# adr-arroyo/PointCloudComparator

Measured on NVIDIA B200. Metric: knn_queries_per_s_k16_10M, higher is better.
Workload: dtype f32

## Files before the change

### pointcloudcomparator_b200/csrc/pcc_knn.cu

```cuda
#include <algorithm>
#include <cmath>
#include <cstring>

#include <cub/device/device_select.cuh>
#include <cub/iterator/counting_input_iterator.cuh>

#include "pcc_internal.h"
#include "pcc_fastknn.cuh"

namespace pcc {

__device__ __forceinline__ bool load_query(const Grid &g, const QueryView &v, int64_t t, float &x, float &y, float &z, int64_t &row, bool &write_empty) {
    write_empty = false;
    if (t >= v.nq) return false;
    if (v.self) { row = rows_query(g, v, t, x, y, z); return true; }
    row = rows_query(g, v, t, x, y, z);
#ifdef PCC_EXP_SEQROWS
    row = t;
#endif
#ifdef PCC_EXP_SEQQ
    { float4 p = __ldg(v.q + t); x = p.x; y = p.y; z = p.z; }
#endif
    if (!finite3(x, y, z) || g.n == 0) { write_empty = true; return false; }
    return true;
}

template <class List>
__device__ __forceinline__ void knn_search(const Grid &g, float x, float y, float z, int k, List &list) {
    const QueryCell c = locate(g, x, y, z);
    int Rin = -1, R = 1;
    for (;;) {
        scan_progressive(g, c, Rin, R, [&]() { return to_cell_units(g, key_d2(list.at(k - 1))); },
                         [&](uint32_t, float4 p) { list.offer(make_key(dist2(x, y, z, p.x, p.y, p.z), __float_as_uint(p.w))); });
        const float cov = covered_d2(g, c, R);
        if (cov == CUDART_INF_F) break;
        const nkey_t kth = list.at(k - 1);
        if (kth != PCC_EMPTY_KEY && key_d2(kth) < cov) break;
        Rin = R; R = next_ring(g, R, key_d2(kth));
    }
}

template <int K>
__device__ __forceinline__ void write_row(const nkey_t (&key)[K], int k, int32_t *__restrict__ oi, float *__restrict__ od, int vec4) {
    if (vec4 && K >= 4 && k == K) {
#pragma unroll
        for (int j = 0; j + 3 < K; j += 4) {
            reinterpret_cast<int4 *>(oi)[j >> 2] = make_int4(key_idx(key[j]), key_idx(key[j + 1]), key_idx(key[j + 2]), key_idx(key[j + 3]));
            reinterpret_cast<float4 *>(od)[j >> 2] = make_float4(key_d2(key[j]), key_d2(key[j + 1]), key_d2(key[j + 2]), key_d2(key[j + 3]));
        }
    } else {
#pragma unroll
        for (int j = 0; j < K; ++j) if (j < k) { oi[j] = key_idx(key[j]); od[j] = key_d2(key[j]); }
    }
}
template <int K>
__device__ __forceinline__ void knn_reg_body(const Grid &g, const QueryView &v, int64_t t, int k, int32_t *__restrict__ out_idx, float *__restrict__ out_d2, int vec4) {
    float x, y, z; int64_t row; bool empty;
    RegList<K> list; list.init();
    const bool live = load_query(g, v, t, x, y, z, row, empty);
    if (!live && !empty) return;
    if (live) knn_search(g, x, y, z, k, list);
    write_row<K>(list.key, k, out_idx + row * k, out_d2 + row * k, vec4);
}
template <int K>
__global__ void __launch_bounds__(128) knn_reg_kernel(Grid g, QueryView v, int k, int32_t *__restrict__ out_idx, float *__restrict__ out_d2, int vec4) {
    knn_reg_body<K>(g, v, (int64_t)blockIdx.x * blockDim.x + threadIdx.x, k, out_idx, out_d2, vec4);
}
constexpr unsigned kTiedToWide = 4096;
struct FixList { uint32_t *list; unsigned *count; unsigned long long *stats; uint32_t *ring_list; unsigned *ring_count; uint8_t *ring_flag; uint32_t *wide_list; unsigned *wide_count; uint32_t *late_list; unsigned *late_count; uint32_t *retry_list; unsigned *retry_count; };
__device__ __forceinline__ void push_list(uint32_t *list, unsigned *count, uint32_t value) {
    const unsigned mask = __activemask();
    const int leader = __ffs(mask) - 1, lane = threadIdx.x & 31;
    unsigned base = 0;
    if (lane == leader) base = atomicAdd(count, (unsigned)__popc(mask));
    base = __shfl_sync(mask, base, leader);
    list[base + __popc(mask & ((1u << lane) - 1))] = value;
}
template <int K>
__global__ void __launch_bounds__(128) knn_fixup_kernel(Grid g, QueryView v, int k, int32_t *__restrict__ out_idx, float *__restrict__ out_d2, int vec4, FixList fix) {
    const unsigned n = *fix.count;
    if (fix.wide_list && n <= kTiedToWide) return;
    for (unsigned i = blockIdx.x * blockDim.x + threadIdx.x; i < n; i += gridDim.x * blockDim.x) knn_reg_body<K>(g, v, (int64_t)fix.list[i], k, out_idx, out_d2, vec4);
}

#ifndef PCC_LOG16
#define PCC_LOG16 48
#endif
#ifndef PCC_MB16
#define PCC_MB16 9
#endif
#ifndef PCC_LOG32
#define PCC_LOG32 80
#endif
#ifndef PCC_MB32
#define PCC_MB32 5
#endif
constexpr int64_t kSmallBatch = 1024, kSmallBatchBigK = 64;
constexpr int kRingMaxR = 3;
template <int K> struct FastCfg { static constexpr int threads = 128, log_slots = K <= 16 ? PCC_LOG16 : PCC_LOG32, min_blocks = K <= 16 ? PCC_MB16 : PCC_MB32; };
}
#include "pcc_knn_thr.cuh"
namespace pcc {
template <int K>
__device__ __forceinline__ float kth_distance(const Grid &g, const QueryCell &c, float x, float y, float z, int k, RegDist<K> &list, bool &proved,
                                              uint32_t *__restrict__ slog, int &nlog, const int R0) {
    scan_progressive(g, c, -1, R0, [&]() { return to_cell_units(g, (k == K) ? list.d[K - 1] : list.at(k - 1)); }, [&](uint32_t pos, float4 p) {
        const float d2 = dist2(x, y, z, p.x, p.y, p.z);
        if (d2 <= list.d[K - 1]) {
            if (nlog < FastCfg<K>::log_slots) slog[nlog * FastCfg<K>::threads] = pos;
            ++nlog;
            list.insert(d2);
        }
    });
    const float kth = (k == K) ? list.d[K - 1] : list.at(k - 1);
    const float cov = covered_d2(g, c, R0);
    proved = cov == CUDART_INF_F || kth < cov;
    return kth;
}
template <int K>
__device__ __forceinline__ void knn_fast_body(const Grid &g, const QueryView &v, const int64_t t, int k, int32_t *__restrict__ out_idx, float *__restrict__ out_d2, int vec4,
                                              const FixList &fix, uint32_t *__restrict__ slog, const int R0) {
    constexpr int kFastThreads = FastCfg<K>::threads, kLogSlots = FastCfg<K>::log_slots;
    float x, y, z; int64_t row; bool empty;
    const bool live = load_query(g, v, t, x, y, z, row, empty);
    if (!live) {
        if (R0 == 1 && t < v.nq) fix.ring_flag[t] = 0;
        if (empty) { nkey_t e[K];
#pragma unroll
            for (int j = 0; j < K; ++j) e[j] = PCC_EMPTY_KEY;
            write_row<K>(e, k, out_idx + row * k, out_d2 + row * k, vec4); }
        return;
    }
    const QueryCell c = locate(g, x, y, z);
    RegDist<K> list; list.init();
    int nlog = 0; bool proved;
    const float tau = kth_distance<K>(g, c, x, y, z, k, list, proved, slog, nlog, R0);
    int m = 0;
    if (nlog <= kLogSlots) {
        for (int i = 0; i < nlog; ++i) {
            const uint32_t pos = slog[i * kFastThreads];
            const float4 p = __ldg(g.pts + pos);
            if (dist2(x, y, z, p.x, p.y, p.z) <= tau) { slog[m * kFastThreads] = pos; ++m; }
        }
    } else {
        scan_clipped(g, c, -1, R0, to_cell_units(g, tau), [&](uint32_t pos, float4 p) {
            if (dist2(x, y, z, p.x, p.y, p.z) <= tau) { if (m < kLogSlots) slog[m * kFastThreads] = pos; ++m; }
        });
    }
    if (fix.stats && R0 == 1) { atomicAdd(fix.stats + 0, 1ull); atomicAdd(fix.stats + 1, (unsigned long long)nlog); atomicAdd(fix.stats + 4, proved ? 0ull : 1ull); atomicAdd(fix.stats + 5, m > K ? 1ull : 0ull); atomicAdd(fix.stats + 6, (unsigned long long)m); atomicAdd(fix.stats + 3, nlog > kLogSlots ? 1ull : 0ull); }
    const bool tied = m > K;
    const bool wide = !tied && !proved && (tau == CUDART_INF_F || next_ring(g, 1, tau) > kRingMaxR);
    if (R0 == 1) fix.ring_flag[t] = (!tied && !proved && !wide) ? 1 : 0;
    if (tied) { push_list(fix.list, fix.count, (uint32_t)t); return; }
    if (wide) { push_list(fix.wide_list, fix.wide_count, (uint32_t)t); return; }
    nkey_t e[K];
#pragma unroll
    for (int j = 0; j < K; ++j) {
        e[j] = PCC_EMPTY_KEY;
        if (j < m) { const float4 p = __ldg(g.pts + slog[j * kFastThreads]); e[j] = make_key(dist2(x, y, z, p.x, p.y, p.z), __float_as_uint(p.w)); }
    }
    bitonic_sort_key<K>(e);
    write_row<K>(e, k, out_idx + row * k, out_d2 + row * k, vec4);
}
template <int K>
__global__ void __launch_bounds__(FastCfg<K>::threads, FastCfg<K>::min_blocks) knn_fast_kernel(Grid g, QueryView v, int k, int32_t *__restrict__ out_idx, float *__restrict__ out_d2, int vec4, FixList fix) {
    __shared__ uint32_t slog_all[FastCfg<K>::log_slots * FastCfg<K>::threads];
    knn_fast_body<K>(g, v, (int64_t)blockIdx.x * blockDim.x + threadIdx.x, k, out_idx, out_d2, vec4, fix, slog_all + threadIdx.x, 1);
}
__device__ __forceinline__ nkey_t warp_sort_keys(nkey_t v, int lane) {
#pragma unroll
    for (int size = 2; size <= 32; size <<= 1) {
#pragma unroll
        for (int j = size >> 1; j > 0; j >>= 1) {
            const nkey_t o = __shfl_xor_sync(0xffffffffu, v, j);
            const bool keep_min = ((lane & j) == 0) == ((lane & size) == 0);
            v = (keep_min == (o < v)) ? o : v;
        }
    }
    return v;
}
__device__ __forceinline__ nkey_t warp_merge_keys(nkey_t best, nkey_t batch, int lane) {
    batch = warp_sort_keys(batch, lane);
    const nkey_t r = __shfl_sync(0xffffffffu, batch, 31 - lane);
    nkey_t v = r < best ? r : best;
#pragma unroll
    for (int j = 16; j > 0; j >>= 1) {
        const nkey_t o = __shfl_xor_sync(0xffffffffu, v, j);
        v = (((lane & j) == 0) == (o < v)) ? o : v;
    }
    return v;
}
constexpr int kWideRuns = 64;
__device__ __forceinline__ uint32_t warp_inclusive_scan(uint32_t v, int lane) {
#pragma unroll
    for (int o = 1; o < 32; o <<= 1) { const uint32_t w = __shfl_up_sync(0xffffffffu, v, o); if (lane >= o) v += w; }
    return v;
}
__global__ void __launch_bounds__(128, 5) knn_wide_kernel(Grid g, QueryView v, int k, int32_t *__restrict__ out_idx, float *__restrict__ out_d2, FixList fix,
                                                         const uint32_t *__restrict__ wlist, const unsigned *__restrict__ wcount, int take_tied) {
    __shared__ uint32_t srun_j[4 * kWideRuns], srun_len[4 * kWideRuns], srun_off[4 * (kWideRuns + 1)];
    const int lane = threadIdx.x & 31, wib = threadIdx.x >> 5;
    uint32_t *run_j = srun_j + wib * kWideRuns, *run_len = srun_len + wib * kWideRuns, *run_off = srun_off + wib * (kWideRuns + 1);
    const unsigned n_wide = *wcount, n_tied = (take_tied && *fix.count <= kTiedToWide) ? *fix.count : 0u, n = n_wide + n_tied;
    const unsigned full = 0xffffffffu, lt = (1u << lane) - 1u;
    for (unsigned i = blockIdx.x * 4 + wib; i < n; i += gridDim.x * 4) {
        float x, y, z; int64_t row; bool empty;
        if (!load_query(g, v, (int64_t)(i < n_wide ? wlist[i] : fix.list[i - n_wide]), x, y, z, row, empty)) continue;
        const QueryCell c = locate(g, x, y, z);
        int Rin = -1, R = 3;
        nkey_t best = PCC_EMPTY_KEY;
        float tau = CUDART_INF_F;
        unsigned long long steps = 0;
        for (;;) {
            const int n1 = 2 * R + 1, nrows = n1 * n1;
            const float tau_u = to_cell_units(g, tau);
            const int per = Rin < 0 ? 2 : 1;
            for (int row0 = 0; row0 < nrows; row0 += 32 * per) {
                RowRuns r; r.j1 = r.e1 = r.j2 = r.e2 = 0;
                if (row0 + lane < nrows) r = row_runs(g, c, Rin, R, tau_u, (row0 + lane) / n1, (row0 + lane) % n1);
                if (per == 2 && row0 + 32 + lane < nrows) {
                    const RowRuns r2 = row_runs(g, c, Rin, R, tau_u, (row0 + 32 + lane) / n1, (row0 + 32 + lane) % n1);
                    r.j2 = r2.j1; r.e2 = r2.e1;
                }
                const unsigned m1 = __ballot_sync(full, r.j1 < r.e1), m2 = __ballot_sync(full, r.j2 < r.e2);
                const int nrun = __popc(m1) + __popc(m2);
                if (nrun == 0) continue;
                if (r.j1 < r.e1) { const int q = __popc(m1 & lt); run_j[q] = r.j1; run_len[q] = r.e1 - r.j1; }
                if (r.j2 < r.e2) { const int q = __popc(m1) + __popc(m2 & lt); run_j[q] = r.j2; run_len[q] = r.e2 - r.j2; }
                __syncwarp();
                const uint32_t la = lane < nrun ? run_len[lane] : 0u, lb = lane + 32 < nrun ? run_len[lane + 32] : 0u;
                const uint32_t ia = warp_inclusive_scan(la, lane), ib = warp_inclusive_scan(lb, lane);
                const uint32_t ta = __shfl_sync(full, ia, 31), P = ta + __shfl_sync(full, ib, 31);
                run_off[lane] = ia - la; run_off[lane + 32] = ta + ib - lb;
                if (lane == 0) run_off[kWideRuns] = P;
                __syncwarp();
                int rc = 0;
                for (uint32_t q0 = 0; q0 < P; q0 += 64) {
                    bool has[2] = {false, false}; nkey_t key[2] = {PCC_EMPTY_KEY, PCC_EMPTY_KEY}; float4 p[2];
#pragma unroll
                    for (int u = 0; u < 2; ++u) {
                        const uint32_t q = q0 + 32 * u + lane;
                        has[u] = q < P;
                        if (has[u]) { while (q >= run_off[rc + 1]) ++rc; p[u] = __ldg(g.pts + run_j[rc] + (q - run_off[rc])); }
                    }
#pragma unroll
                    for (int u = 0; u < 2; ++u) {
                        if (has[u]) { const float d2 = dist2(x, y, z, p[u].x, p[u].y, p[u].z); has[u] = d2 <= tau; key[u] = has[u] ? make_key(d2, __float_as_uint(p[u].w)) : PCC_EMPTY_KEY; }
                        if (__ballot_sync(full, has[u])) {
                            best = warp_merge_keys(best, key[u], lane);
                            tau = key_d2(__shfl_sync(full, best, k - 1));
                        }
                    }
                    ++steps;
                }
                __syncwarp();
            }
            const float cov = covered_d2(g, c, R);
            if (cov == CUDART_INF_F || tau < cov) break;
            Rin = R; R = next_ring(g, R, tau);
        }
        if (fix.stats && lane == 0) { atomicAdd(fix.stats + 2, 1ull); atomicAdd(fix.stats + 7, steps); atomicAdd(fix.stats + 8 + (R <= 1 ? 0 : R == 2 ? 1 : R == 3 ? 2 : R < 8 ? 3 : R < 16 ? 4 : 5), 1ull); }
        if (lane < k) { out_idx[row * k + lane] = key_idx(best); out_d2[row * k + lane] = key_d2(best); }
        __syncwarp();
    }
}
constexpr int kRingLog = 24, kRingRuns = 12;
#ifndef PCC_RINGS_MB
#define PCC_RINGS_MB 6
#endif
template <int K>
__global__ void __launch_bounds__(128, K <= 16 ? PCC_RINGS_MB : 4) knn_rings_kernel(Grid g, QueryView v, int k, int32_t *__restrict__ out_idx, float *__restrict__ out_d2, int vec4, FixList fix) {
    __shared__ uint32_t slog_all[kRingLog * 128];
    __shared__ uint2 srun_all[kRingRuns * 128];
    uint32_t *slog = slog_all + threadIdx.x;
    uint2 *srun = srun_all + threadIdx.x;
    const unsigned n = *fix.ring_count;
    for (unsigned i = blockIdx.x * blockDim.x + threadIdx.x; i < n; i += gridDim.x * blockDim.x) {
        const uint32_t t = fix.ring_list[i];
        float x, y, z; int64_t row; bool empty;
        if (!load_query(g, v, (int64_t)t, x, y, z, row, empty)) continue;
        int32_t *oi = out_idx + row * k; float *od = out_d2 + row * k;
        float kth = od[k - 1];
        const QueryCell c = locate(g, x, y, z);
        const int R = kth == CUDART_INF_F ? kRingMaxR + 1 : next_ring(g, 1, kth);
        bool defer = R > kRingMaxR;
        int ncand = 0, nrun = 0, nlog = 0;
        if (!defer) {
            const float tau_u = to_cell_units(g, kth), rad = sqrtf(tau_u) + 2e-3f;
            const int z0 = max(max(c.cz - R, 0), (int)floorf(c.uz - rad)), z1 = min(min(c.cz + R, g.nz - 1), (int)floorf(c.uz + rad));
            const int y0 = max(max(c.cy - R, 0), (int)floorf(c.uy - rad)), y1 = min(min(c.cy + R, g.ny - 1), (int)floorf(c.uy + rad));
            for (int zz = z0; zz <= z1; ++zz) {
                const float gz = fmaxf(fmaxf((float)zz - c.uz, c.uz - (float)(zz + 1)) - 2e-3f, 0.f);
                for (int yy = y0; yy <= y1; ++yy) {
                    const float gy = fmaxf(fmaxf((float)yy - c.uy, c.uy - (float)(yy + 1)) - 2e-3f, 0.f);
                    const float D = gy * gy + gz * gz;
                    if (D > tau_u) continue;
                    const float w = sqrtf(tau_u - D) + 2e-3f;
                    const int xlo = max(max(c.cx - R, 0), (int)floorf(c.ux - w)), xhi = min(min(c.cx + R, g.nx - 1), (int)floorf(c.ux + w));
                    const uint32_t base = (uint32_t)(((size_t)zz * g.ny + yy) * g.nx);
                    const bool shell = max(abs(zz - c.cz), abs(yy - c.cy)) > 1;
                    const int xa1 = xlo, xb1 = shell ? xhi : min(xhi, c.cx - 2);
                    const int xa2 = max(xlo, c.cx + 2), xb2 = shell ? -1 : xhi;
                    if (xa1 <= xb1) { if (ncand < kRingLog) slog[ncand * 128] = (base + (uint32_t)xa1) | ((uint32_t)(xb1 - xa1) << 28); ++ncand; }
                    if (xa2 <= xb2) { if (ncand < kRingLog) slog[ncand * 128] = (base + (uint32_t)xa2) | ((uint32_t)(xb2 - xa2) << 28); ++ncand; }
                }
            }
            defer = ncand > kRingLog;
        }
        if (!defer) {
            for (int r0 = 0; r0 < ncand; r0 += 4) {
                uint32_t cw[4], w0[4], w1[4];
#pragma unroll
                for (int u = 0; u < 4; ++u) {
                    cw[u] = slog[min(r0 + u, ncand - 1) * 128];
                    const uint32_t b = cw[u] & 0x0fffffffu;
                    w0[u] = __ldg(g.occ + (b >> 5)); w1[u] = __ldg(g.occ + (b >> 5) + 1);
                }
#pragma unroll
                for (int u = 0; u < 4; ++u) {
                    const uint32_t b = cw[u] & 0x0fffffffu, len = (cw[u] >> 28) + 1u;
                    const uint32_t bits = __funnelshift_r(w0[u], w1[u], b & 31u) & ((1u << len) - 1u);
                    if (r0 + u < ncand && bits != 0u) { if (nrun < kRingRuns) srun[nrun * 128] = make_uint2(b, b + len); ++nrun; }
                }
            }
            defer = nrun > kRingRuns;
        }
        if (!defer && nrun > 0) {
            for (int r0 = 0; r0 < nrun; r0 += 4) {
                uint2 pr[4];
#pragma unroll
                for (int u = 0; u < 4; ++u) { const uint2 cr = srun[min(r0 + u, nrun - 1) * 128]; pr[u] = make_uint2(__ldg(g.cell_start + cr.x), __ldg(g.cell_start + cr.y)); }
#pragma unroll
                for (int u = 0; u < 4; ++u) if (r0 + u < nrun) srun[(r0 + u) * 128] = pr[u];
            }
            int r = 0;
// ... 397 lines not shown
    p[0] = v.x; p[1] = v.y; p[2] = v.z;
}

__global__ void fill_f32_kernel(float *p, int64_t n, float v) { int64_t i = (int64_t)blockIdx.x * blockDim.x + threadIdx.x; if (i < n) p[i] = v; }

template <int K>
static void launch_knn_reg(const Grid &g, const QueryView &v, int k, int32_t *oi, float *od, int vec4, cudaStream_t s) {
    knn_reg_kernel<K><<<nblocks(v.nq, 128), 128, 0, s>>>(g, v, k, oi, od, vec4);
    PCC_LAUNCHED();
}
template <int K>
static void launch_knn_cell(const Grid &g, const QueryView &v, int k, int32_t *oi, float *od, int vec4, FixList fix, cudaStream_t s) {
    fix.wide_list = nullptr;
    cudaMemsetAsync(fix.count, 0, sizeof(unsigned), s);
    knn_cell_kernel<K><<<nblocks(v.nq, kCellWarps * 32), kCellWarps * 32, 0, s>>>(g, v, k, oi, od, vec4, fix);
    PCC_LAUNCHED();
    knn_fixup_kernel<K><<<148 * 4, 128, 0, s>>>(g, v, k, oi, od, vec4, fix);
    PCC_LAUNCHED();
}
constexpr int64_t kCalibSample = 1 << 15;
constexpr float kCalibQuantile = 0.99f;
template <int K>
static int calibrate_thr(pcc_index *idx, const Grid &g, const QueryView &v, int k, cudaStream_t s) {
    PCC_TRY(idx->calib.reserve((size_t)kCalibBuckets * kCalibBins * 4 + kCalibBuckets * 4));
    unsigned *hist = idx->calib.as<unsigned>();
    float *ratio = (float *)(hist + kCalibBuckets * kCalibBins);
    PCC_CUDA(cudaMemsetAsync(hist, 0, (size_t)kCalibBuckets * kCalibBins * 4, s));
    const int64_t stride = std::max<int64_t>(1, v.nq / kCalibSample), ns = (v.nq + stride - 1) / stride;
    knn_calib_kernel<K><<<nblocks(ns, 128), 128, 0, s>>>(g, v, k, stride, hist);
    PCC_LAUNCHED();
    static const float quantile = getenv("PCC_THR_QUANTILE") ? (float)atof(getenv("PCC_THR_QUANTILE")) : kCalibQuantile;
    knn_calib_finish_kernel<<<1, kCalibBuckets, 0, s>>>(hist, ratio, quantile);
    PCC_LAUNCHED();
    return PCC_OK;
}
template <int K>
static int launch_knn_fast(pcc_index *idx, const Grid &g, const QueryView &v, int k, int32_t *oi, float *od, int vec4, FixList fix, cudaStream_t s) {
    size_t tmp = idx->sel_tmp_bytes;
    if (idx->sel_tmp_nq != v.nq) {
        cub::DeviceSelect::Flagged(nullptr, tmp, cub::CountingInputIterator<uint32_t>(0), fix.ring_flag, fix.ring_list, fix.ring_count, (int)v.nq, s);
        idx->sel_tmp_nq = v.nq; idx->sel_tmp_bytes = tmp;
    }
    PCC_TRY(idx->cub_tmp.reserve(tmp));
    if (!idx->aux_stream) {
        PCC_CUDA(cudaStreamCreateWithFlags(&idx->aux_stream, cudaStreamNonBlocking));
        PCC_CUDA(cudaEventCreateWithFlags(&idx->ev_fork, cudaEventDisableTiming));
        PCC_CUDA(cudaEventCreateWithFlags(&idx->ev_join, cudaEventDisableTiming));
    }
    if (fix.stats) { cudaMemsetAsync(fix.count, 0, sizeof(unsigned), s); cudaMemsetAsync(fix.wide_count, 0, 3 * sizeof(unsigned), s); }
    else cudaMemsetAsync(fix.count, 0, 33 * sizeof(unsigned), s);
    static const bool old_fast_env = getenv("PCC_OLD_FAST") != nullptr;
    static const bool thr_all = getenv("PCC_THR_ALL") != nullptr;
    const bool old_fast = old_fast_env || (K != 16 && !thr_all) || v.nq >= (1ll << 31);
    if (old_fast) {
        knn_fast_kernel<K><<<nblocks(v.nq, FastCfg<K>::threads), FastCfg<K>::threads, 0, s>>>(g, v, k, oi, od, vec4, fix);
        PCC_LAUNCHED();
    } else {
        const pcc_index *owner = idx->grid_owner ? idx->grid_owner : idx;
        unsigned *h_fb = (unsigned *)((char *)idx->h_pinned + 2048);
        if (idx->calib_k == k && idx->calib_gen == owner->grid_gen && idx->calib_nq > 0 && (double)h_fb[0] > 0.04 * (double)idx->calib_nq) idx->calib_k = -1;
        if (idx->calib_k != k || idx->calib_gen != owner->grid_gen) {
            PCC_TRY(calibrate_thr<K>(idx, g, v, k, s));
            idx->calib_k = k; idx->calib_gen = owner->grid_gen;
        }
        const float *ratio = (const float *)(idx->calib.as<unsigned>() + kCalibBuckets * kCalibBins);
        static std::atomic<unsigned long long> attr_done{0};
        if (!((attr_done.load() >> (idx->device & 63)) & 1ull)) {
            PCC_CUDA(cudaFuncSetAttribute(knn_thr_kernel<K, true>, cudaFuncAttributeMaxDynamicSharedMemorySize, (int)ThrCfg<K>::smem));
            PCC_CUDA(cudaFuncSetAttribute(knn_thr_kernel<K, false>, cudaFuncAttributeMaxDynamicSharedMemorySize, (int)ThrCfg<K>::smem));
            PCC_CUDA(cudaFuncSetAttribute(knn_thr_retry_kernel<K, true>, cudaFuncAttributeMaxDynamicSharedMemorySize, (int)ThrCfg<K>::smem));
            PCC_CUDA(cudaFuncSetAttribute(knn_thr_retry_kernel<K, false>, cudaFuncAttributeMaxDynamicSharedMemorySize, (int)ThrCfg<K>::smem));
            attr_done.fetch_or(1ull << (idx->device & 63));
        }
        const char *staged_env = getenv("PCC_THR_STAGED");
        const bool staged = staged_env && atoi(staged_env) != 0;
        if (staged && k == K) {
            static std::atomic<unsigned long long> sattr_done{0};
            if (!((sattr_done.load() >> (idx->device & 63)) & 1ull)) {
                PCC_CUDA(cudaFuncSetAttribute(knn_thr_staged_kernel<K, true>, cudaFuncAttributeMaxDynamicSharedMemorySize, (int)ThrStagedCfg<K>::smem));
                sattr_done.fetch_or(1ull << (idx->device & 63));
            }
            knn_thr_staged_kernel<K, true><<<nblocks(v.nq, ThrCfg<K>::threads), ThrCfg<K>::threads, ThrStagedCfg<K>::smem, s>>>(g, v, k, oi, od, vec4, fix, ratio);
            PCC_LAUNCHED();
            knn_thr_retry_kernel<K, true><<<148 * 4, ThrCfg<K>::threads, ThrCfg<K>::smem, s>>>(g, v, k, oi, od, vec4, fix, ratio);
            PCC_LAUNCHED();
        } else if (k == K) {
            knn_thr_kernel<K, true><<<nblocks(v.nq, ThrCfg<K>::threads), ThrCfg<K>::threads, ThrCfg<K>::smem, s>>>(g, v, k, oi, od, vec4, fix, ratio);
            PCC_LAUNCHED();
            knn_thr_retry_kernel<K, true><<<148 * 4, ThrCfg<K>::threads, ThrCfg<K>::smem, s>>>(g, v, k, oi, od, vec4, fix, ratio);
            PCC_LAUNCHED();
        } else {
            knn_thr_kernel<K, false><<<nblocks(v.nq, ThrCfg<K>::threads), ThrCfg<K>::threads, ThrCfg<K>::smem, s>>>(g, v, k, oi, od, vec4, fix, ratio);
            PCC_LAUNCHED();
            knn_thr_retry_kernel<K, false><<<148 * 4, ThrCfg<K>::threads, ThrCfg<K>::smem, s>>>(g, v, k, oi, od, vec4, fix, ratio);
            PCC_LAUNCHED();
        }
        h_fb[0] = 0; idx->calib_nq = v.nq;
        PCC_CUDA(cudaMemcpyAsync(h_fb, fix.retry_count, sizeof(unsigned), cudaMemcpyDeviceToHost, s));
    }
    PCC_CUDA(cudaEventRecord(idx->ev_fork, s));
    PCC_CUDA(cudaStreamWaitEvent(idx->aux_stream, idx->ev_fork, 0));
    knn_wide_kernel<<<148 * 6, 128, 0, idx->aux_stream>>>(g, v, k, oi, od, fix, fix.wide_list, fix.wide_count, old_fast ? 1 : 0);
    PCC_LAUNCHED();
    PCC_CUDA(cudaEventRecord(idx->ev_join, idx->aux_stream));
    PCC_CUDA(cub::DeviceSelect::Flagged(idx->cub_tmp.p, tmp, cub::CountingInputIterator<uint32_t>(0), fix.ring_flag, fix.ring_list, fix.ring_count, (int)v.nq, s));
    PCC_LAUNCHED();
    knn_rings_kernel<K><<<148 * 16, 128, 0, s>>>(g, v, k, oi, od, vec4, fix);
    PCC_LAUNCHED();
    PCC_CUDA(cudaStreamWaitEvent(s, idx->ev_join, 0));
    knn_wide_kernel<<<148 * 2, 128, 0, s>>>(g, v, k, oi, od, fix, fix.late_list, fix.late_count, 0);
    PCC_LAUNCHED();
    if (old_fast) {
        knn_fixup_kernel<K><<<148 * 4, 128, 0, s>>>(g, v, k, oi, od, vec4, fix);
        PCC_LAUNCHED();
    }
    return PCC_OK;
}

}

using namespace pcc;

static int knn_impl(pcc_index *idx, const void *q, int64_t nq, int stride_bytes, int k, int32_t *out_idx, float *out_d2, int *k_eff, int mem, cudaStream_t s, bool sync) {
    Queries qs;
    PCC_TRY(prepare_queries(idx, q, nq, stride_bytes, mem, s, &qs));
    if (k_eff) *k_eff = (int)std::min<int64_t>(k, idx->n_indexed);
    if (qs.rows == 0) return PCC_OK;
    if (!out_idx || !out_d2) return fail(PCC_ERR_INVALID, "output pointers are NULL");
    int32_t *oi = out_idx; float *od = out_d2;
    const size_t cells = (size_t)qs.rows * k;
    if (mem == PCC_HOST) {
        PCC_TRY(idx->out_i.reserve(cells * 4)); PCC_TRY(idx->out_f.reserve(cells * 4));
        oi = idx->out_i.as<int32_t>(); od = idx->out_f.as<float>();
    }
    if (qs.self && !idx->all_rows_indexed) {
        PCC_CUDA(cudaMemsetAsync(oi, 0xFF, cells * 4, s));
        fill_f32_kernel<<<nblocks((int64_t)cells, 256), 256, 0, s>>>(od, (int64_t)cells, INFINITY);
        PCC_LAUNCHED();
    }
    const Grid g = idx->grid();
    const QueryView v = view_of(qs);
    const int vec4 = ((((uintptr_t)oi) | ((uintptr_t)od)) & 15) == 0 && (k % 4 == 0);
    KernelTimer timer(idx, s);
    if (qs.nq > 0) {
        static const bool exact_env = getenv("PCC_EXACT_ONLY") != nullptr;
        const bool exact_only = exact_env || v.nq < (k <= 32 ? kSmallBatch : kSmallBatchBigK);
        static const bool want_stats = getenv("PCC_STATS") != nullptr;
        const char *cell_env = getenv("PCC_CELL_KERNEL");
        const bool use_cell = cell_env && atoi(cell_env) != 0;
        FixList fix{nullptr, nullptr, nullptr, nullptr, nullptr, nullptr, nullptr, nullptr, nullptr, nullptr, nullptr, nullptr};
        if (k > 1 && k <= 32 && !exact_only) {
            PCC_TRY(idx->misc.reserve((size_t)v.nq * 21 + 512));
            fix.count = idx->misc.as<unsigned>(); fix.ring_count = fix.count + 1; fix.wide_count = fix.count + 30; fix.late_count = fix.count + 31; fix.retry_count = fix.count + 32;
            fix.list = idx->misc.as<uint32_t>() + 64; fix.ring_list = fix.list + v.nq; fix.wide_list = fix.ring_list + v.nq; fix.late_list = fix.wide_list + v.nq; fix.retry_list = fix.late_list + v.nq; fix.ring_flag = (uint8_t *)(fix.retry_list + v.nq);
            if (want_stats) { fix.stats = (unsigned long long *)(idx->misc.as<uint32_t>() + 2); PCC_CUDA(cudaMemsetAsync(fix.stats, 0, 112, s)); }
        }
        if (k == 1) launch_knn_reg<1>(g, v, k, oi, od, vec4, s);
        else if (exact_only && k <= 2) launch_knn_reg<2>(g, v, k, oi, od, vec4, s);
        else if (exact_only && k <= 4) launch_knn_reg<4>(g, v, k, oi, od, vec4, s);
        else if (exact_only && k <= 8) launch_knn_reg<8>(g, v, k, oi, od, vec4, s);
        else if (exact_only && k <= 16) launch_knn_reg<16>(g, v, k, oi, od, vec4, s);
        else if (exact_only && k <= 32) launch_knn_reg<32>(g, v, k, oi, od, vec4, s);
        else if (use_cell && k <= 8) launch_knn_cell<8>(g, v, k, oi, od, vec4, fix, s);
        else if (use_cell && k <= 16) launch_knn_cell<16>(g, v, k, oi, od, vec4, fix, s);
        else if (use_cell && k <= 32) launch_knn_cell<32>(g, v, k, oi, od, vec4, fix, s);
        else if (k <= 4) PCC_TRY(launch_knn_fast<4>(idx, g, v, k, oi, od, vec4, fix, s));
        else if (k <= 8) PCC_TRY(launch_knn_fast<8>(idx, g, v, k, oi, od, vec4, fix, s));
        else if (k <= 16) PCC_TRY(launch_knn_fast<16>(idx, g, v, k, oi, od, vec4, fix, s));
        else if (k <= 32) PCC_TRY(launch_knn_fast<32>(idx, g, v, k, oi, od, vec4, fix, s));
        else if (!exact_only) PCC_TRY(knn_select(idx, qs, k, oi, od, s));
        else {
            const int th = heap_threads(k);
            PCC_TRY(set_heap_smem(knn_heap_kernel));
            knn_heap_kernel<<<nblocks(v.nq, th), th, (size_t)k * th * sizeof(nkey_t), s>>>(g, v, k, oi, od);
            PCC_LAUNCHED();
        }
        PCC_CUDA(cudaGetLastError());
    }
    timer.stop();
    if (getenv("PCC_STATS") && k > 1 && k <= 32) {
        unsigned long long h[14];
        cudaMemcpyAsync(h, idx->misc.as<uint32_t>() + 2, 112, cudaMemcpyDeviceToHost, s); cudaStreamSynchronize(s);
        const double q = (double)std::max<unsigned long long>(h[0], 1);
        fprintf(stderr, "[pcc stats] queries=%llu logged/q=%.1f log_overflow=%.5f need_ring2=%.3f fixup=%.5f members/q=%.2f\n",
                h[0], h[1] / q, h[3] / q, h[4] / q, h[5] / q, h[6] / q);
        fprintf(stderr, "[pcc stats] wide queries=%llu steps/q=%.1f final R: <=1 %llu, 2 %llu, 3 %llu, 4-7 %llu, 8-15 %llu, 16+ %llu\n", h[2], h[7] / (double)std::max<unsigned long long>(h[2], 1), h[8], h[9], h[10], h[11], h[12], h[13]);
    }
    if (mem == PCC_HOST) {
        PCC_TRY(copy_out(out_idx, oi, cells * 4, mem, s));
        PCC_TRY(copy_out(out_d2, od, cells * 4, mem, s));
        if (sync) PCC_CUDA(cudaStreamSynchronize(s));
    }
    return PCC_OK;
}

extern "C" {

int pcc_knn(pcc_index *idx, const void *q, int64_t nq, int stride_bytes, int k, int32_t *out_idx, float *out_d2, int *k_eff, int mem, void *stream) {
    PCC_TRY(check_index(idx, stream));
    if (k < 1 || k > PCC_MAX_K) return fail(PCC_ERR_INVALID, "k=%d outside 1..%d", k, PCC_MAX_K);
    cudaStream_t s = (cudaStream_t)stream;
    static const int64_t kChunk = getenv("PCC_PIPE_CHUNK_LOG2") ? (1ll << std::max(16, std::min(24, atoi(getenv("PCC_PIPE_CHUNK_LOG2"))))) : (1ll << 20);
    if (mem == PCC_HOST && q && nq >= 2 * kChunk && !idx->timing && stride_bytes >= 12 && !(stride_bytes & 3)) {
        if (!out_idx || !out_d2) return fail(PCC_ERR_INVALID, "output pointers are NULL");
        if (!idx->shadow) {
            idx->shadow = new pcc_index();
            idx->shadow->device = idx->device;
// ... 159 lines not shown
```

### pointcloudcomparator_b200/csrc/pcc_knn_thr.cuh

```cuda
#pragma once
#include <utility>

#include "pcc_device.cuh"

namespace pcc {

#ifndef PCC_THR_QAHEAD
#define PCC_THR_QAHEAD 0
#endif
#ifndef PCC_THR_EARLY
#define PCC_THR_EARLY 16
#endif
#ifndef PCC_THR_JOINT
#define PCC_THR_JOINT 1
#endif
#ifndef PCC_THR_SLOTS8
#define PCC_THR_SLOTS8 36
#endif
#ifndef PCC_THR_SLOTS16
#define PCC_THR_SLOTS16 48
#endif
#ifndef PCC_THR_SLOTS32
#define PCC_THR_SLOTS32 100
#endif
// ... 173 lines not shown
    if (j < e) {
        const float4 p0 = load_pt<GEN>(pts, j), p1 = load_pt<GEN>(pts, min(j + 1, e - 1)), p2 = load_pt<GEN>(pts, min(j + 2, e - 1));
        const float d0 = dist2(x, y, z, p0.x, p0.y, p0.z), d1 = dist2(x, y, z, p1.x, p1.y, p1.z), d2 = dist2(x, y, z, p2.x, p2.y, p2.z);
        sts_v2(wa, __float_as_uint(d0), j); advance_if_le<STRIDE>(wa, d0, tau);
        sts_v2(wa, __float_as_uint(d1), j + 1); advance_if_le_and<STRIDE>(wa, d1, tau, j + 1 < e);
        sts_v2(wa, __float_as_uint(d2), j + 2); advance_if_le_and<STRIDE>(wa, d2, tau, j + 2 < e);
        dmin = fminf(fminf(dmin, d0), fminf(d1, d2)); tau = dmin + T;
        if (!COMPRESS) wa = min(wa, cap);
        else if (PCC_THR_JOINT ? __any_sync(__activemask(), wa >= cap) : (wa >= cap)) on_full();
    }
}

constexpr float kRetryScale = 4.f;
#ifndef PCC_THR_TILE
#define PCC_THR_TILE 384
#endif
namespace thr_tma {
__device__ __forceinline__ uint32_t smem_u32(const void *p) { return (uint32_t)__cvta_generic_to_shared(p); }
__device__ __forceinline__ void mbar_init(unsigned long long *bar, unsigned count) {
    asm volatile("mbarrier.init.shared::cta.b64 [%0], %1;" ::"r"(smem_u32(bar)), "r"(count) : "memory");
    asm volatile("fence.mbarrier_init.release.cluster;" ::: "memory");
}
__device__ __forceinline__ void mbar_expect_tx(unsigned long long *bar, unsigned bytes) {
    asm volatile("mbarrier.arrive.expect_tx.shared::cta.b64 _, [%0], %1;" ::"r"(smem_u32(bar)), "r"(bytes) : "memory");
}
__device__ __forceinline__ void bulk_g2s(void *dst, const void *src, unsigned bytes, unsigned long long *bar) {
    asm volatile("cp.async.bulk.shared::cluster.global.mbarrier::complete_tx::bytes [%0], [%1], %2, [%3];"
                 ::"r"(smem_u32(dst)), "l"(src), "r"(bytes), "r"(smem_u32(bar)) : "memory");
}
__device__ __forceinline__ void mbar_wait(unsigned long long *bar, unsigned parity) {
    asm volatile("{\n\t.reg .pred p;\n\tWAIT_%=:\n\tmbarrier.try_wait.parity.shared::cta.b64 p, [%0], %1;\n\t@p bra DONE_%=;\n\tbra WAIT_%=;\n\tDONE_%=:\n\t}"
                 ::"r"(smem_u32(bar)), "r"(parity) : "memory");
}
}
#ifndef PCC_THR_MAIN_COMPRESS
#define PCC_THR_MAIN_COMPRESS 0
#endif
template <int K, bool FULLK, bool RETRY, bool STAGED = false, bool COMPRESS = RETRY>
__device__ __forceinline__ void knn_thr_body(const Grid &g, const QueryView &v, const int64_t t, const int k_rt, int32_t *__restrict__ out_idx, float *__restrict__ out_d2, int vec4,
                                             const FixList &fix, const float *__restrict__ ratio, uint2 *__restrict__ slog, const bool loose = false,
                                             float4 *tile = nullptr, unsigned long long *bar = nullptr) {
    constexpr int TH = ThrCfg<K>::threads, SLOTS = ThrCfg<K>::slots, B = ThrCfg<K>::B;
    constexpr uint32_t SMASK = (1u << ThrCfg<K>::slot_bits) - 1u;
    const int k = FULLK ? K : k_rt;
    float x = 0.f, y = 0.f, z = 0.f; int64_t row = 0; bool empty = false;
#if PCC_THR_QAHEAD
    uint32_t qi_ahead = 0xFFFFFFFFu;
    if (!RETRY && !STAGED && v.order) {
        constexpr int64_t AHEAD = (int64_t)PCC_THR_QAHEAD * ThrCfg<K>::threads;
        if ((threadIdx.x & 31) == 0 && t + 2 * AHEAD < v.nq) prefetch_l2(v.order + t + 2 * AHEAD);
        if (t + AHEAD < v.nq) qi_ahead = __ldg(v.order + t + AHEAD);
    }
#endif
    const bool live = load_query(g, v, t, x, y, z, row, empty);
    auto leave_dead = [&]() {
        if (t < v.nq) fix.ring_flag[t] = 0;
        if (empty) { nkey_t e[K];
#pragma unroll
            for (int j = 0; j < K; ++j) e[j] = PCC_EMPTY_KEY;
            write_row<K>(e, k, out_idx + row * k, out_d2 + row * k, vec4); }
    };
    if (!STAGED && !live) { leave_dead(); return; }
    QueryCell c; c.cx = c.cy = c.cz = 0; c.ux = c.uy = c.uz = 0.f;
    if (live) c = locate(g, x, y, z);
    uint32_t M = 0, s0 = 0, e0 = 0, rowmask = 0;
    if (live) {
        const int xa = max(c.cx - 1, 0), xb = min(c.cx + 1, g.nx - 1);
        uint32_t rs[9], re[9];
#pragma unroll
        for (int r = 0; r < 9; ++r) {
            const int zz = c.cz + centre_out(r / 3), yy = c.cy + centre_out(r % 3);
            rs[r] = re[r] = 0;
            if (zz >= 0 && zz < g.nz && yy >= 0 && yy < g.ny) {
                const size_t rowb = ((size_t)zz * g.ny + yy) * g.nx;
                rs[r] = cell_begin(g, rowb + xa); re[r] = cell_begin(g, rowb + xb + 1);
            }
        }
#pragma unroll
        for (int r = 0; r < 9; ++r) { M += re[r] - rs[r]; rowmask |= (re[r] > rs[r] ? 1u : 0u) << r; if (!STAGED && (PCC_THR_PREFETCH & 1)) prefetch_run<3, false>(g.pts, rs[r], re[r]); }
        s0 = rs[0]; e0 = re[0];
    }
#if PCC_THR_QAHEAD
    if (!RETRY && !STAGED && qi_ahead != 0xFFFFFFFFu) prefetch_l2(v.q + qi_ahead);
#endif
    auto leave_wide = [&]() {
        fix.ring_flag[t] = 0;
        if (fix.stats) { atomicAdd(fix.stats + 0, 1ull); atomicAdd(fix.stats + 4, 1ull); }
        push_list(fix.wide_list, fix.wide_count, (uint32_t)t);
    };
    const bool walker = live && M >= (uint32_t)k;
    if (!STAGED && !walker) { leave_wide(); return; }
    bool lane_staged = false;
    uint32_t my_start = 0, my_off = 0;
    if (STAGED) {
        const unsigned full = 0xffffffffu;
        const int lane = threadIdx.x & 31;
        const unsigned wmask = __ballot_sync(full, walker);
        if (wmask) {
            const int leader = __ffs(wmask) - 1;
            const int lcy = __shfl_sync(full, c.cy, leader), lcz = __shfl_sync(full, c.cz, leader);
            bool inrow = walker && c.cy == lcy && c.cz == lcz;
            const int xmin = __reduce_min_sync(full, inrow ? c.cx : 0x7fffffff);
            inrow = inrow && c.cx <= xmin + 9;
            const int xmax = __reduce_max_sync(full, inrow ? c.cx : xmin);
            uint32_t len = 0;
            if (lane < 9) {
                const int zz = lcz + centre_out(lane / 3), yy = lcy + centre_out(lane % 3);
// ... 41 lines not shown
            oem_sort_u32<B>(blk);
            merge_prune_u32<B>(best, blk, dropmin);
        }
    };
    auto kth_key = [&]() {
        uint32_t kth = best[K - 1];
        if (!FULLK) {
            kth = 0u;
            static_for<K - 1>([&](auto I) { constexpr int i = decltype(I)::value; kth = max(kth, i < k ? best[i] : 0u); });
        }
        return kth;
    };
    bool give_up = false;
    auto compress_if = [&](const int min_n) {
        const int nf = (int)((wa - wa0) / STRIDE);
        if (nf < min_n) return;
        select_log(nf);
        const float tau_new = __uint_as_float(slog[(kth_key() & SMASK) * TH].x) * (1.f + 1.f / 32768.f);
        if (tau_new < tau) { dmin = 0.f; T = tau_new; tau = tau_new; }
        int m = 0;
        for (int i = 0; i < nf; ++i) { const uint2 e = slog[i * TH]; if (__uint_as_float(e.x) <= tau) { slog[m * TH] = e; ++m; } }
        if (m >= LOGCAP - 4) { give_up = true; m = 0; }
        wa = wa0 + (uint32_t)m * STRIDE;
    };
    auto on_full = [&]() { compress_if(wa >= cap ? 0 : K + 13); };
    {
        const RowRuns none = {0u, 0u, 0u, 0u};
        int az = 0, ay = 0;
        if (!walker) rowmask = 0;
        RowRuns nxt = (rowmask & 1u) ? row_runs(g, c, -1, 1, to_cell_units(g, tau), 0, 0) : none;
        for (;;) {
            const RowRuns cur = nxt;
            const int r = az * 3 + ay;
            if (++ay == 3) { ay = 0; ++az; }
            const bool more = az < 3;
            nxt = none;
            if (more && ((rowmask >> (az * 3 + ay)) & 1u)) { nxt = row_runs(g, c, -1, 1, to_cell_units(g, tau), az, ay); if (!STAGED && (PCC_THR_PREFETCH & 2)) prefetch_run<3, true>(g.pts, nxt.j1, nxt.e1); }
            if (STAGED) {
                const uint32_t st = __shfl_sync(0xffffffffu, my_start, r), of = __shfl_sync(0xffffffffu, my_off, r);
                const float4 *src = lane_staged ? (const float4 *)tile + of - st : g.pts;
                thr_walk_run<STRIDE, COMPRESS, true>(src, cur.j1, cur.e1, x, y, z, T, dmin, tau, wa, cap, on_full);
            } else thr_walk_run<STRIDE, COMPRESS, false>(g.pts, cur.j1, cur.e1, x, y, z, T, dmin, tau, wa, cap, on_full);
            (void)r;
            if (!more) break;
            if (COMPRESS && PCC_THR_EARLY > 0) {
                const int nl = (int)((wa - wa0) / STRIDE);
                if (__any_sync(__activemask(), nl >= LOGCAP - PCC_THR_EARLY)) compress_if(K + 5);
            }
        }
    }
    if (STAGED && !live) { leave_dead(); return; }
    if (STAGED && !walker) { leave_wide(); return; }
    if (RETRY && give_up) { fix.ring_flag[t] = 0; knn_reg_body<K>(g, v, t, k, out_idx, out_d2, vec4); return; }
    if (!RETRY && COMPRESS && give_up) { fix.ring_flag[t] = 0; push_list(fix.retry_list, fix.retry_count, (uint32_t)t); return; }
    const int n = (int)((wa - wa0) / STRIDE);
    select_log(n);
    const uint32_t kth = kth_key();
    uint32_t gap = 0xFFFFFFFFu;
    static_for<K>([&](auto I) {
        constexpr int i = decltype(I)::value;
        const uint32_t nxt = i + 1 < B ? best[i + 1] : dropmin;
        const uint32_t d = nxt - best[i];
        gap = min(gap, (FULLK || i < k) ? d : 0xFFFFFFFFu);
    });
    const bool overflow = n >= LOGCAP;
    const bool tie = kth == 0xFFFFFFFFu || gap <= SMASK;
    float tau_k = CUDART_INF_F;
    if (kth != 0xFFFFFFFFu) tau_k = __uint_as_float(slog[(kth & SMASK) * TH].x);
    const bool under = !(tau_k <= tau);
    if (fix.stats && !RETRY) { atomicAdd(fix.stats + 0, 1ull); atomicAdd(fix.stats + 1, (unsigned long long)n); atomicAdd(fix.stats + 3, overflow ? 1ull : 0ull); atomicAdd(fix.stats + 5, (overflow || tie || under) ? 1ull : 0ull); atomicAdd(fix.stats + 6, (unsigned long long)M); }
    if (!RETRY && (overflow || tie || under)) {
        fix.ring_flag[t] = 0;
        push_list(fix.retry_list, fix.retry_count, (uint32_t)t | ((under && !overflow) ? 0x80000000u : 0u));
        return;
    }
    int32_t *oi = out_idx + row * k; float *od = out_d2 + row * k;
    if (RETRY && (overflow || tie || under)) {
        RegList<K> list; list.init();
        if (!overflow) for (int i = 0; i < n; ++i) { const uint2 e = slog[i * TH]; list.offer(((nkey_t)e.x << 32) | __float_as_uint(__ldg(&g.pts[e.y].w))); }
        const nkey_t kk = FULLK ? list.key[K - 1] : list.at(k - 1);
        tau_k = key_d2(kk);
        if (overflow || kk == PCC_EMPTY_KEY || !(tau_k <= tau)) { fix.ring_flag[t] = 0; knn_reg_body<K>(g, v, t, k, out_idx, out_d2, vec4); return; }
        const float cov = covered_d2(g, c, 1);
        const bool proved = cov == CUDART_INF_F || tau_k < cov;
        const bool wide = !proved && next_ring(g, 1, tau_k) > kRingMaxR;
        fix.ring_flag[t] = (!proved && !wide) ? 1 : 0;
        if (wide) { push_list(fix.wide_list, fix.wide_count, (uint32_t)t); return; }
        write_row<K>(list.key, k, oi, od, vec4);
        return;
    }
    const float cov = covered_d2(g, c, 1);
    const bool proved = cov == CUDART_INF_F || tau_k < cov;
    const bool wide = !proved && next_ring(g, 1, tau_k) > kRingMaxR;
    if (fix.stats && !RETRY) atomicAdd(fix.stats + 4, proved ? 0ull : 1ull);
    fix.ring_flag[t] = (!proved && !wide) ? 1 : 0;
    if (wide) { push_list(fix.wide_list, fix.wide_count, (uint32_t)t); return; }
    static_for<K / 4>([&](auto Q) {
        constexpr int q = decltype(Q)::value * 4;
        uint2 le[4]; int32_t id[4];
        static_for<4>([&](auto I) { constexpr int i = decltype(I)::value; le[i] = (FULLK || q + i < k) ? slog[(best[q + i] & SMASK) * TH] : make_uint2(0u, 0u); });
        static_for<4>([&](auto I) { constexpr int i = decltype(I)::value; id[i] = __float_as_int(__ldg(&g.pts[le[i].y].w)); });
        if (FULLK && vec4) {
            __stcs(reinterpret_cast<int4 *>(oi) + (q >> 2), make_int4(id[0], id[1], id[2], id[3]));
            __stcs(reinterpret_cast<float4 *>(od) + (q >> 2), make_float4(__uint_as_float(le[0].x), __uint_as_float(le[1].x), __uint_as_float(le[2].x), __uint_as_float(le[3].x)));
        } else {
            static_for<4>([&](auto I) { constexpr int i = decltype(I)::value; if (q + i < k) { oi[q + i] = id[i]; od[q + i] = __uint_as_float(le[i].x); } });
        }
    });
}
template <int K, bool FULLK>
__global__ void __launch_bounds__(ThrCfg<K>::threads, ThrCfg<K>::min_blocks) knn_thr_kernel(Grid g, QueryView v, int k, int32_t *__restrict__ out_idx, float *__restrict__ out_d2, int vec4, FixList fix, const float *__restrict__ ratio) {
    extern __shared__ uint2 thr_log[];
    knn_thr_body<K, FULLK, false, false, PCC_THR_MAIN_COMPRESS != 0>(g, v, (int64_t)blockIdx.x * blockDim.x + threadIdx.x, k, out_idx, out_d2, vec4, fix, ratio, thr_log + threadIdx.x);
}
#ifndef PCC_THR_STAGED_MB
#define PCC_THR_STAGED_MB 3
#endif
template <int K> struct ThrStagedCfg {
    static constexpr int warps = ThrCfg<K>::threads / 32;
    static constexpr size_t log_bytes = ThrCfg<K>::smem, tile_bytes = (size_t)warps * PCC_THR_TILE * sizeof(float4);
    static constexpr size_t smem = log_bytes + tile_bytes + warps * sizeof(unsigned long long);
};
template <int K, bool FULLK>
__global__ void __launch_bounds__(ThrCfg<K>::threads, PCC_THR_STAGED_MB) knn_thr_staged_kernel(Grid g, QueryView v, int k, int32_t *__restrict__ out_idx, float *__restrict__ out_d2, int vec4, FixList fix, const float *__restrict__ ratio) {
    extern __shared__ __align__(128) unsigned char thr_smem[];
    uint2 *log = reinterpret_cast<uint2 *>(thr_smem);
    float4 *tiles = reinterpret_cast<float4 *>(thr_smem + ThrStagedCfg<K>::log_bytes);
    unsigned long long *bars = reinterpret_cast<unsigned long long *>(thr_smem + ThrStagedCfg<K>::log_bytes + ThrStagedCfg<K>::tile_bytes);
    const int warp = threadIdx.x >> 5;
    if ((threadIdx.x & 31) == 0) thr_tma::mbar_init(bars + warp, 1);
    __syncwarp();
    knn_thr_body<K, FULLK, false, true>(g, v, (int64_t)blockIdx.x * blockDim.x + threadIdx.x, k, out_idx, out_d2, vec4, fix, ratio, log + threadIdx.x, false,
                                        tiles + (size_t)warp * PCC_THR_TILE, bars + warp);
}
template <int K, bool FULLK>
__global__ void __launch_bounds__(ThrCfg<K>::threads, 2) knn_thr_retry_kernel(Grid g, QueryView v, int k, int32_t *__restrict__ out_idx, float *__restrict__ out_d2, int vec4, FixList fix, const float *__restrict__ ratio) {
    extern __shared__ uint2 thr_log[];
    const unsigned n = *fix.retry_count;
    for (unsigned i = blockIdx.x * blockDim.x + threadIdx.x; i < n; i += gridDim.x * blockDim.x) {
        const uint32_t e = fix.retry_list[i];
        knn_thr_body<K, FULLK, true>(g, v, (int64_t)(e & 0x7FFFFFFFu), k, out_idx, out_d2, vec4, fix, ratio, thr_log + threadIdx.x, (e >> 31) != 0u);
    }
}

}
```

Baseline: 2.655 billion.

## Fork wide-search kernel earlier and hand off query coords to later stages

Launches the wide-radius kernel on the auxiliary stream right after the main kNN kernel, so it overlaps the retry, compaction and ring stages. Retry-produced wide queries now go to the late list, and the join with the auxiliary stream moves to the end. Stages also write each query's coordinates, kth distance and output row into a compact hand-off buffer. Later kernels read that buffer instead of re-gathering the query point and reading back the written distance row, at the cost of more scratch memory and extra stores.

```diff
diff --git a/pointcloudcomparator_b200/csrc/pcc_knn.cu b/pointcloudcomparator_b200/csrc/pcc_knn.cu
--- a/pointcloudcomparator_b200/csrc/pcc_knn.cu
+++ b/pointcloudcomparator_b200/csrc/pcc_knn.cu
@@ -67,7 +67,12 @@
     knn_reg_body<K>(g, v, (int64_t)blockIdx.x * blockDim.x + threadIdx.x, k, out_idx, out_d2, vec4);
 }
 constexpr unsigned kTiedToWide = 4096;
-struct FixList { uint32_t *list; unsigned *count; unsigned long long *stats; uint32_t *ring_list; unsigned *ring_count; uint8_t *ring_flag; uint32_t *wide_list; unsigned *wide_count; uint32_t *late_list; unsigned *late_count; uint32_t *retry_list; unsigned *retry_count; };
+struct FixList { uint32_t *list; unsigned *count; unsigned long long *stats; uint32_t *ring_list; unsigned *ring_count; uint8_t *ring_flag; uint32_t *wide_list; unsigned *wide_count; uint32_t *late_list; unsigned *late_count; uint32_t *retry_list; unsigned *retry_count;
+                 float4 *hand; uint32_t *hand_row; };
+__device__ __forceinline__ void hand_off(const FixList &fix, int64_t t, float x, float y, float z, float kth, int64_t row) {
+    fix.hand[t] = make_float4(x, y, z, kth);
+    fix.hand_row[t] = (uint32_t)row;
+}
 __device__ __forceinline__ void push_list(uint32_t *list, unsigned *count, uint32_t value) {
     const unsigned mask = __activemask();
     const int leader = __ffs(mask) - 1, lane = threadIdx.x & 31;
@@ -161,6 +166,7 @@
     }
     bitonic_sort_key<K>(e);
     write_row<K>(e, k, out_idx + row * k, out_d2 + row * k, vec4);
+    if (R0 == 1 && !proved) hand_off(fix, t, x, y, z, tau, row);
 }
 template <int K>
 __global__ void __launch_bounds__(FastCfg<K>::threads, FastCfg<K>::min_blocks) knn_fast_kernel(Grid g, QueryView v, int k, int32_t *__restrict__ out_idx, float *__restrict__ out_d2, int vec4, FixList fix) {
@@ -197,7 +203,7 @@
     return v;
 }
 __global__ void __launch_bounds__(128, 5) knn_wide_kernel(Grid g, QueryView v, int k, int32_t *__restrict__ out_idx, float *__restrict__ out_d2, FixList fix,
-                                                         const uint32_t *__restrict__ wlist, const unsigned *__restrict__ wcount, int take_tied) {
+                                                         const uint32_t *__restrict__ wlist, const unsigned *__restrict__ wcount, int take_tied, int from_hand) {
     __shared__ uint32_t srun_j[4 * kWideRuns], srun_len[4 * kWideRuns], srun_off[4 * (kWideRuns + 1)];
     const int lane = threadIdx.x & 31, wib = threadIdx.x >> 5;
     uint32_t *run_j = srun_j + wib * kWideRuns, *run_len = srun_len + wib * kWideRuns, *run_off = srun_off + wib * (kWideRuns + 1);
@@ -205,7 +211,9 @@
     const unsigned full = 0xffffffffu, lt = (1u << lane) - 1u;
     for (unsigned i = blockIdx.x * 4 + wib; i < n; i += gridDim.x * 4) {
         float x, y, z; int64_t row; bool empty;
-        if (!load_query(g, v, (int64_t)(i < n_wide ? wlist[i] : fix.list[i - n_wide]), x, y, z, row, empty)) continue;
+        const uint32_t t = i < n_wide ? wlist[i] : fix.list[i - n_wide];
+        if (from_hand) { const float4 h = fix.hand[t]; x = h.x; y = h.y; z = h.z; row = fix.hand_row[t]; }
+        else if (!load_query(g, v, (int64_t)t, x, y, z, row, empty)) continue;
         const QueryCell c = locate(g, x, y, z);
         int Rin = -1, R = 3;
         nkey_t best = PCC_EMPTY_KEY;
@@ -277,10 +285,11 @@
     const unsigned n = *fix.ring_count;
     for (unsigned i = blockIdx.x * blockDim.x + threadIdx.x; i < n; i += gridDim.x * blockDim.x) {
         const uint32_t t = fix.ring_list[i];
-        float x, y, z; int64_t row; bool empty;
-        if (!load_query(g, v, (int64_t)t, x, y, z, row, empty)) continue;
+        const float4 h = fix.hand[t];
+        const float x = h.x, y = h.y, z = h.z;
+        float kth = h.w;
+        const int64_t row = fix.hand_row[t];
         int32_t *oi = out_idx + row * k; float *od = out_d2 + row * k;
-        float kth = od[k - 1];
         const QueryCell c = locate(g, x, y, z);
         const int R = kth == CUDART_INF_F ? kRingMaxR + 1 : next_ring(g, 1, kth);
         bool defer = R > kRingMaxR;
@@ -784,9 +793,18 @@
     static const bool old_fast_env = getenv("PCC_OLD_FAST") != nullptr;
     static const bool thr_all = getenv("PCC_THR_ALL") != nullptr;
     const bool old_fast = old_fast_env || (K != 16 && !thr_all) || v.nq >= (1ll << 31);
+    auto fork_wide = [&]() -> int {
+        PCC_CUDA(cudaEventRecord(idx->ev_fork, s));
+        PCC_CUDA(cudaStreamWaitEvent(idx->aux_stream, idx->ev_fork, 0));
+        knn_wide_kernel<<<148 * 6, 128, 0, idx->aux_stream>>>(g, v, k, oi, od, fix, fix.wide_list, fix.wide_count, old_fast ? 1 : 0, 0);
+        PCC_LAUNCHED();
+        PCC_CUDA(cudaEventRecord(idx->ev_join, idx->aux_stream));
+        return PCC_OK;
+    };
     if (old_fast) {
         knn_fast_kernel<K><<<nblocks(v.nq, FastCfg<K>::threads), FastCfg<K>::threads, 0, s>>>(g, v, k, oi, od, vec4, fix);
         PCC_LAUNCHED();
+        PCC_TRY(fork_wide());
     } else {
         const pcc_index *owner = idx->grid_owner ? idx->grid_owner : idx;
         unsigned *h_fb = (unsigned *)((char *)idx->h_pinned + 2048);
@@ -814,38 +832,36 @@
             }
             knn_thr_staged_kernel<K, true><<<nblocks(v.nq, ThrCfg<K>::threads), ThrCfg<K>::threads, ThrStagedCfg<K>::smem, s>>>(g, v, k, oi, od, vec4, fix, ratio);
             PCC_LAUNCHED();
+            PCC_TRY(fork_wide());
             knn_thr_retry_kernel<K, true><<<148 * 4, ThrCfg<K>::threads, ThrCfg<K>::smem, s>>>(g, v, k, oi, od, vec4, fix, ratio);
             PCC_LAUNCHED();
         } else if (k == K) {
             knn_thr_kernel<K, true><<<nblocks(v.nq, ThrCfg<K>::threads), ThrCfg<K>::threads, ThrCfg<K>::smem, s>>>(g, v, k, oi, od, vec4, fix, ratio);
             PCC_LAUNCHED();
+            PCC_TRY(fork_wide());
             knn_thr_retry_kernel<K, true><<<148 * 4, ThrCfg<K>::threads, ThrCfg<K>::smem, s>>>(g, v, k, oi, od, vec4, fix, ratio);
             PCC_LAUNCHED();
         } else {
             knn_thr_kernel<K, false><<<nblocks(v.nq, ThrCfg<K>::threads), ThrCfg<K>::threads, ThrCfg<K>::smem, s>>>(g, v, k, oi, od, vec4, fix, ratio);
             PCC_LAUNCHED();
+            PCC_TRY(fork_wide());
             knn_thr_retry_kernel<K, false><<<148 * 4, ThrCfg<K>::threads, ThrCfg<K>::smem, s>>>(g, v, k, oi, od, vec4, fix, ratio);
             PCC_LAUNCHED();
         }
         h_fb[0] = 0; idx->calib_nq = v.nq;
         PCC_CUDA(cudaMemcpyAsync(h_fb, fix.retry_count, sizeof(unsigned), cudaMemcpyDeviceToHost, s));
     }
-    PCC_CUDA(cudaEventRecord(idx->ev_fork, s));
-    PCC_CUDA(cudaStreamWaitEvent(idx->aux_stream, idx->ev_fork, 0));
-    knn_wide_kernel<<<148 * 6, 128, 0, idx->aux_stream>>>(g, v, k, oi, od, fix, fix.wide_list, fix.wide_count, old_fast ? 1 : 0);
-    PCC_LAUNCHED();
-    PCC_CUDA(cudaEventRecord(idx->ev_join, idx->aux_stream));
     PCC_CUDA(cub::DeviceSelect::Flagged(idx->cub_tmp.p, tmp, cub::CountingInputIterator<uint32_t>(0), fix.ring_flag, fix.ring_list, fix.ring_count, (int)v.nq, s));
     PCC_LAUNCHED();
     knn_rings_kernel<K><<<148 * 16, 128, 0, s>>>(g, v, k, oi, od, vec4, fix);
     PCC_LAUNCHED();
-    PCC_CUDA(cudaStreamWaitEvent(s, idx->ev_join, 0));
-    knn_wide_kernel<<<148 * 2, 128, 0, s>>>(g, v, k, oi, od, fix, fix.late_list, fix.late_count, 0);
+    knn_wide_kernel<<<148 * 2, 128, 0, s>>>(g, v, k, oi, od, fix, fix.late_list, fix.late_count, 0, 1);
     PCC_LAUNCHED();
     if (old_fast) {
         knn_fixup_kernel<K><<<148 * 4, 128, 0, s>>>(g, v, k, oi, od, vec4, fix);
         PCC_LAUNCHED();
     }
+    PCC_CUDA(cudaStreamWaitEvent(s, idx->ev_join, 0));
     return PCC_OK;
 }
 
@@ -880,11 +896,12 @@
         static const bool want_stats = getenv("PCC_STATS") != nullptr;
         const char *cell_env = getenv("PCC_CELL_KERNEL");
         const bool use_cell = cell_env && atoi(cell_env) != 0;
-        FixList fix{nullptr, nullptr, nullptr, nullptr, nullptr, nullptr, nullptr, nullptr, nullptr, nullptr, nullptr, nullptr};
+        FixList fix{nullptr, nullptr, nullptr, nullptr, nullptr, nullptr, nullptr, nullptr, nullptr, nullptr, nullptr, nullptr, nullptr, nullptr};
         if (k > 1 && k <= 32 && !exact_only) {
-            PCC_TRY(idx->misc.reserve((size_t)v.nq * 21 + 512));
+            PCC_TRY(idx->misc.reserve((size_t)v.nq * 41 + 512));
             fix.count = idx->misc.as<unsigned>(); fix.ring_count = fix.count + 1; fix.wide_count = fix.count + 30; fix.late_count = fix.count + 31; fix.retry_count = fix.count + 32;
-            fix.list = idx->misc.as<uint32_t>() + 64; fix.ring_list = fix.list + v.nq; fix.wide_list = fix.ring_list + v.nq; fix.late_list = fix.wide_list + v.nq; fix.retry_list = fix.late_list + v.nq; fix.ring_flag = (uint8_t *)(fix.retry_list + v.nq);
+            fix.hand = (float4 *)(idx->misc.as<uint32_t>() + 64); fix.hand_row = (uint32_t *)(fix.hand + v.nq);
+            fix.list = fix.hand_row + v.nq; fix.ring_list = fix.list + v.nq; fix.wide_list = fix.ring_list + v.nq; fix.late_list = fix.wide_list + v.nq; fix.retry_list = fix.late_list + v.nq; fix.ring_flag = (uint8_t *)(fix.retry_list + v.nq);
             if (want_stats) { fix.stats = (unsigned long long *)(idx->misc.as<uint32_t>() + 2); PCC_CUDA(cudaMemsetAsync(fix.stats, 0, 112, s)); }
         }
         if (k == 1) launch_knn_reg<1>(g, v, k, oi, od, vec4, s);
diff --git a/pointcloudcomparator_b200/csrc/pcc_knn_thr.cuh b/pointcloudcomparator_b200/csrc/pcc_knn_thr.cuh
--- a/pointcloudcomparator_b200/csrc/pcc_knn_thr.cuh
+++ b/pointcloudcomparator_b200/csrc/pcc_knn_thr.cuh
@@ -249,7 +249,9 @@
         if (t + AHEAD < v.nq) qi_ahead = __ldg(v.order + t + AHEAD);
     }
 #endif
-    const bool live = load_query(g, v, t, x, y, z, row, empty);
+    bool live;
+    if (RETRY) { const float4 h = fix.hand[t]; x = h.x; y = h.y; z = h.z; row = fix.hand_row[t]; live = true; }
+    else live = load_query(g, v, t, x, y, z, row, empty);
     auto leave_dead = [&]() {
         if (t < v.nq) fix.ring_flag[t] = 0;
         if (empty) { nkey_t e[K];
@@ -397,7 +399,7 @@
     if (STAGED && !live) { leave_dead(); return; }
     if (STAGED && !walker) { leave_wide(); return; }
     if (RETRY && give_up) { fix.ring_flag[t] = 0; knn_reg_body<K>(g, v, t, k, out_idx, out_d2, vec4); return; }
-    if (!RETRY && COMPRESS && give_up) { fix.ring_flag[t] = 0; push_list(fix.retry_list, fix.retry_count, (uint32_t)t); return; }
+    if (!RETRY && COMPRESS && give_up) { fix.ring_flag[t] = 0; hand_off(fix, t, x, y, z, CUDART_INF_F, row); push_list(fix.retry_list, fix.retry_count, (uint32_t)t); return; }
     const int n = (int)((wa - wa0) / STRIDE);
     select_log(n);
     const uint32_t kth = kth_key();
@@ -416,6 +418,7 @@
     if (fix.stats && !RETRY) { atomicAdd(fix.stats + 0, 1ull); atomicAdd(fix.stats + 1, (unsigned long long)n); atomicAdd(fix.stats + 3, overflow ? 1ull : 0ull); atomicAdd(fix.stats + 5, (overflow || tie || under) ? 1ull : 0ull); atomicAdd(fix.stats + 6, (unsigned long long)M); }
     if (!RETRY && (overflow || tie || under)) {
         fix.ring_flag[t] = 0;
+        hand_off(fix, t, x, y, z, CUDART_INF_F, row);
         push_list(fix.retry_list, fix.retry_count, (uint32_t)t | ((under && !overflow) ? 0x80000000u : 0u));
         return;
     }
@@ -430,7 +433,8 @@
         const bool proved = cov == CUDART_INF_F || tau_k < cov;
         const bool wide = !proved && next_ring(g, 1, tau_k) > kRingMaxR;
         fix.ring_flag[t] = (!proved && !wide) ? 1 : 0;
-        if (wide) { push_list(fix.wide_list, fix.wide_count, (uint32_t)t); return; }
+        if (wide) { push_list(fix.late_list, fix.late_count, (uint32_t)t); return; }
+        if (!proved) hand_off(fix, t, x, y, z, tau_k, row);
         write_row<K>(list.key, k, oi, od, vec4);
         return;
     }
@@ -439,7 +443,8 @@
     const bool wide = !proved && next_ring(g, 1, tau_k) > kRingMaxR;
     if (fix.stats && !RETRY) atomicAdd(fix.stats + 4, proved ? 0ull : 1ull);
     fix.ring_flag[t] = (!proved && !wide) ? 1 : 0;
-    if (wide) { push_list(fix.wide_list, fix.wide_count, (uint32_t)t); return; }
+    if (wide) { if (RETRY) push_list(fix.late_list, fix.late_count, (uint32_t)t); else push_list(fix.wide_list, fix.wide_count, (uint32_t)t); return; }
+    if (!proved) hand_off(fix, t, x, y, z, tau_k, row);
     static_for<K / 4>([&](auto Q) {
         constexpr int q = decltype(Q)::value * 4;
         uint2 le[4]; int32_t id[4];
```

After: 2.707 billion, median of 6. +1.9%, better.
